# apache/tez

Hardware: NVIDIA H100
Metric: sorted KV GB/s (16B key / 64B val) (higher is better)
Workload: dtype u8

## Files before the change

### tez_b200/csrc/emit_fast.cuh

```cuda
#pragma once
#include "sorter_kernels.cuh"

#ifndef TEZGPU_EMIT_MIN_CTAS
#define TEZGPU_EMIT_MIN_CTAS 4
#endif

namespace tezgpu {

constexpr int FE_THREADS = 256;
constexpr int FE_MAX_RECS = 256;
constexpr int FE_IMG_BYTES = 22016;

struct TileDesc {
  uint32_t p;
  uint32_t r0;
  uint32_t nr;
  uint32_t flags;
  uint64_t abs0;
  uint64_t after;
};

struct TileCrc {
  uint32_t raw;
  uint32_t p;
  uint64_t after;
};

__global__ void k_build_tiles(EmitParams e, TileDesc *__restrict__ tiles) {
  uint32_t tile = blockIdx.x * blockDim.x + threadIdx.x;
  if (tile >= e.tile_start[e.P]) return;
  int lo = 0, hi = e.P;
  while (hi - lo > 1) {
    int mid = (lo + hi) >> 1;
    if (e.tile_start[mid] <= tile) lo = mid; else hi = mid;
  }
  const uint32_t p = (uint32_t)lo;
  const uint32_t ps = e.part_start[p], pe = e.part_start[p + 1];
  const uint32_t k = tile - e.tile_start[p];
  TileDesc d;
  d.p = p;
  d.r0 = ps + k * e.recs_per_tile;
  d.nr = min(e.recs_per_tile, pe - d.r0);
  const bool first = (k == 0), last = (d.r0 + d.nr == pe);
  d.flags = (first ? 1u : 0u) | (last ? 2u : 0u);
  const uint64_t seg0 = e.seg_start[p];
  d.abs0 = seg0 + (first ? 0 : 4 + (uint64_t)(d.r0 - ps) * e.rec_size);
  const uint64_t tile_end = seg0 + 4 + (uint64_t)(d.r0 - ps + d.nr) * e.rec_size + (last ? 2 : 0);
  d.after = (e.seg_start[p + 1] - 4) - tile_end;
  tiles[tile] = d;
}

__global__ void k_crc_combine(const TileCrc *__restrict__ tc, uint32_t ntiles, const CrcTables *__restrict__ t,
                              uint32_t *__restrict__ seg_crc) {
  uint32_t i = blockIdx.x * blockDim.x + threadIdx.x;
  const int lane = threadIdx.x & 31;
  uint32_t p = 0xFFFFFFFFu, val = 0;
  if (i < ntiles) {
    TileCrc c = tc[i];
    p = c.p;
    val = c.raw ? crc_shift_bytes(t, c.raw, c.after) : 0u;
  }
#pragma unroll
  for (int o = 1; o < 32; o <<= 1) {
    uint32_t v2 = __shfl_up_sync(0xffffffffu, val, o), p2 = __shfl_up_sync(0xffffffffu, p, o);
    if (lane >= o && p2 == p) val ^= v2;
  }
  uint32_t pn = __shfl_down_sync(0xffffffffu, p, 1);
  if (p != 0xFFFFFFFFu && (lane == 31 || pn != p) && val) atomicXor(&seg_crc[p], val);
}

__device__ __forceinline__ void sts_b8(uint32_t a, uint32_t v) { asm volatile("st.shared.b8 [%0], %1;" ::"r"(a), "r"(v) : "memory"); }
__device__ __forceinline__ void sts_b16(uint32_t a, uint32_t v) { asm volatile("st.shared.b16 [%0], %1;" ::"r"(a), "h"((unsigned short)v) : "memory"); }
// ... 32 lines not shown

__device__ __forceinline__ uint4 ldg_stream_v4(const void *p) {
  uint4 r;
  asm volatile("ld.global.nc.L1::no_allocate.v4.u32 {%0,%1,%2,%3}, [%4];"
               : "=r"(r.x), "=r"(r.y), "=r"(r.z), "=r"(r.w) : "l"(p));
  return r;
}
__device__ __forceinline__ void stg_stream_v4(void *p, uint4 v) {
  asm volatile("st.global.L1::no_allocate.v4.u32 [%0], {%1,%2,%3,%4};" ::"l"(p), "r"(v.x), "r"(v.y), "r"(v.z), "r"(v.w) : "memory");
}

struct FastEmitParams {
  EmitParams e;
  const TileDesc *tiles;
  TileCrc *tile_crc;
  uint32_t ntiles;
  uint32_t cpr;
  uint32_t cpr_magic;
  uint32_t stride;
};

__device__ __forceinline__ uint64_t fast_source_offset(const Records &rec, uint32_t ri, uint32_t stride, uint32_t p) {
  if (rec.use_runs) return run_record_off_p(rec.runs, p, ri) + rec.runs.hdr_len;
  return rec.key_off ? rec.key_off[ri] : (uint64_t)ri * stride;
}

template <int UNROLL, bool ALIGNED>
__global__ void __launch_bounds__(FE_THREADS, TEZGPU_EMIT_MIN_CTAS) k_emit_fast(FastEmitParams fp) {
  __shared__ __align__(16) uint8_t s_img[FE_IMG_BYTES];
  __shared__ uint32_t s_idx[2][FE_MAX_RECS];
  __shared__ uint64_t s_off[ALIGNED ? 1 : 2][ALIGNED ? 1 : FE_MAX_RECS];
// ... 5 lines not shown
  const int tid = threadIdx.x, lane = tid & 31, warp = tid >> 5;
  for (int i = tid; i < 4 * 256; i += FE_THREADS) {
    s_tab[i] = (&e.crc->slice[0][0])[i];
    s_adv32[i] = (&e.crc->adv128[0][0])[i];
  }
  const uint32_t lane_pow = e.crc->pow_word[4 * (31 - lane)];
  WarpLinearMap m_word, m_skip;
  {
    const uint32_t *gt = &e.crc->slice[0][0], *ga = &e.crc->advc[0][0];
    m_word.init([&](uint32_t x) { return gt[768 + (x & 0xFF)] ^ gt[512 + ((x >> 8) & 0xFF)] ^ gt[256 + ((x >> 16) & 0xFF)] ^ gt[x >> 24]; }, lane);
    m_skip.init([&](uint32_t x) { return ga[x & 0xFF] ^ ga[256 + ((x >> 8) & 0xFF)] ^ ga[512 + ((x >> 16) & 0xFF)] ^ ga[768 + (x >> 24)]; }, lane);
  }
  const uint32_t img_base = (uint32_t)__cvta_generic_to_shared(s_img);
  const uint8_t *__restrict__ kv = e.rec.kv;
  const uint8_t *kv_end = kv + e.rec.kv_bytes;
  const uint32_t rec_size = e.rec_size, hdr_len = e.fixed_hdr_len, stride = fp.stride;

  TileDesc td_next;
  if (blockIdx.x < fp.ntiles) {
    td_next = fp.tiles[blockIdx.x];
    if ((uint32_t)tid < td_next.nr) {
      const uint32_t ri = e.order[td_next.r0 + tid];
      s_idx[0][tid] = ri;
      if (!ALIGNED) s_off[0][tid] = fast_source_offset(e.rec, ri, stride, td_next.p);
    }
  }
  uint32_t buf = 0;
  for (uint32_t tile = blockIdx.x; tile < fp.ntiles; tile += gridDim.x, buf ^= 1u) {
    const TileDesc td = td_next;
    const uint32_t nr = td.nr;
    const bool first_tile = td.flags & 1u, last_tile = td.flags & 2u;
    const uint32_t tile_n = tile + gridDim.x;
    if (tile_n < fp.ntiles) td_next = fp.tiles[tile_n];
    __syncthreads();
    const uint32_t *__restrict__ c_idx = s_idx[buf];
    const uint64_t *__restrict__ c_off = s_off[ALIGNED ? 0 : buf];
    const uint64_t abs0 = td.abs0;
    const uint32_t lead = (uint32_t)(abs0 & 15u);
    const uint32_t rec0 = lead + (first_tile ? 4u : 0u);
    const uint32_t body_end = rec0 + nr * rec_size + (last_tile ? 2u : 0u);

    const uint32_t npieces = nr * fp.cpr;
    const uint32_t half_up = (nr + 1) >> 1;
    for (uint32_t q0 = tid; q0 < npieces; q0 += FE_THREADS * UNROLL) {
      uint4 v[UNROLL];
      uint32_t dst[UNROLL];
#pragma unroll
      for (int u = 0; u < UNROLL; u++) {
// ... 18 lines not shown
              case 2: w0 = lo4.z; w1 = lo4.w; w2 = hi4.x; w3 = hi4.y; w4 = hi4.z; break;
              default: w0 = lo4.w; w1 = hi4.x; w2 = hi4.y; w3 = hi4.z; w4 = hi4.w; break;
            }
            v[u] = make_uint4(__funnelshift_r(w0, w1, bsh), __funnelshift_r(w1, w2, bsh), __funnelshift_r(w2, w3, bsh),
                              __funnelshift_r(w3, w4, bsh));
          }
          dst[u] = img_base + rec0 + j * rec_size + hdr_len + 16u * c;
        }
      }
#pragma unroll
      for (int u = 0; u < UNROLL; u++) {
        uint32_t q = q0 + u * FE_THREADS;
        if (q < npieces) sts16_unaligned(dst[u], v[u]);
      }
    }
    if (tile_n < fp.ntiles && (uint32_t)tid < td_next.nr) {
      const uint32_t ri = e.order[td_next.r0 + tid];
      s_idx[buf ^ 1u][tid] = ri;
      if (!ALIGNED) s_off[buf ^ 1u][tid] = fast_source_offset(e.rec, ri, stride, td_next.p);
    }
    if ((uint32_t)tid < nr) {
      uint32_t a = img_base + rec0 + tid * rec_size;
      for (uint32_t b = 0; b < hdr_len; b++) sts_b8(a + b, e.fixed_hdr[b]);
    }
    if (tid == 0) {
      if (first_tile) { s_img[lead] = 'T'; s_img[lead + 1] = 'I'; s_img[lead + 2] = 'F'; s_img[lead + 3] = 0; }
      if (last_tile) { s_img[body_end - 2] = 0xFF; s_img[body_end - 1] = 0xFF; }
    }
    __syncthreads();

    const uint32_t cb0 = rec0, cb1 = body_end;
// ... 71 lines not shown
```

### tez_b200/csrc/emit_pipe.cuh

```cuda
#pragma once
#include "emit_fast.cuh"

#ifndef TEZGPU_EMIT4_MIN_CTAS
#define TEZGPU_EMIT4_MIN_CTAS 3
#endif

namespace tezgpu {

constexpr int FE4_BATCH = FE_THREADS / 32;
constexpr int FE4_UNROLL = 5;
constexpr int FE4_RUN = 5;
constexpr uint32_t FE4_RUN_BYTES = 16u * FE4_RUN;
constexpr int FE4_IMG_BYTES = FE_THREADS * FE4_RUN * 16;
constexpr int FE4_GROUPS = 2;
constexpr int FE4_PARKED = 4;
constexpr int FE4_WBITS = 7;
constexpr int FE4_WDIGITS = (32 + FE4_WBITS - 1) / FE4_WBITS;
constexpr int FE4_WENTRIES = ((FE4_WDIGITS - 1) << FE4_WBITS) + (1 << (32 - FE4_WBITS * (FE4_WDIGITS - 1)));

static inline uint32_t emit4_max_recs(uint32_t rec_size) {
  return std::min<uint32_t>(FE_MAX_RECS, (FE4_IMG_BYTES - 15 - 4 - 2) / rec_size);
}

constexpr uint32_t FE4_MAX_CPR = 8;
// ... 47 lines not shown
  using L = Emit4Smem;
  constexpr int BATCH = FE4_PARKED;
  extern __shared__ __align__(16) uint8_t smem4[];
  uint32_t *s_wtab = reinterpret_cast<uint32_t *>(smem4);
  uint32_t *s_tab = reinterpret_cast<uint32_t *>(smem4 + L::WTAB);
  uint32_t *s_hor = s_tab + 256;
  const int sub = threadIdx.x / FE_THREADS, tid = threadIdx.x % FE_THREADS, lane = tid & 31, warp = tid >> 5;
  uint8_t *gbase = smem4 + L::SHARED + (size_t)sub * L::GROUP;
  uint8_t *s_img = gbase;
  uint32_t(*s_idx)[FE_MAX_RECS] = reinterpret_cast<uint32_t(*)[FE_MAX_RECS]>(gbase + FE4_IMG_BYTES);
  uint32_t(*s_part)[FE_THREADS] = reinterpret_cast<uint32_t(*)[FE_THREADS]>(gbase + FE4_IMG_BYTES + 3 * FE_MAX_RECS * 4);
  FoldMeta *s_meta = reinterpret_cast<FoldMeta *>(gbase + FE4_IMG_BYTES + 3 * FE_MAX_RECS * 4 + (size_t)BATCH * FE_THREADS * 4);
  auto group_sync = [&]() { asm volatile("bar.sync %0, %1;" ::"r"(sub + 1), "r"(FE_THREADS) : "memory"); };

  const EmitParams &e = fp.e;
  const uint32_t G = gridDim.x * FE4_GROUPS, ntiles = fp.ntiles;
  uint32_t tile = blockIdx.x * FE4_GROUPS + sub;
  for (int i = threadIdx.x; i < FE4_WENTRIES * 32; i += FE_THREADS * FE4_GROUPS)
    s_wtab[i] = emit4_wtab_value(e.crc, (uint32_t)(i >> 5) >> FE4_WBITS, (uint32_t)(i >> 5) & ((1u << FE4_WBITS) - 1));
  for (int i = threadIdx.x; i < 256; i += FE_THREADS * FE4_GROUPS) s_tab[i] = e.crc->slice[0][i];
  {
    const uint32_t x_hor = e.crc->pow0[FE4_RUN_BYTES * 32];
    for (int i = threadIdx.x; i < 4 * 256; i += FE_THREADS * FE4_GROUPS) s_hor[i] = crc_multmodp((uint32_t)(i & 255) << (8 * (i >> 8)), x_hor);
  }
  __syncthreads();
  if (tile >= ntiles) return;
  const uint32_t lane_pow = e.crc->pow0[FE4_RUN_BYTES * (31 - lane)];
  const uint8_t *wt = reinterpret_cast<const uint8_t *>(s_wtab + lane);
  auto next_word = [&](uint32_t x) -> uint32_t { return emit4_next_word(wt, x); };
  const uint32_t img_base = (uint32_t)__cvta_generic_to_shared(s_img);
  const uint8_t *__restrict__ kv = e.rec.kv;
// ... 191 lines not shown
```

### tez_b200/csrc/emit_pipe_u.cuh

```cuda
#pragma once
#include "emit_pipe.cuh"

namespace tezgpu {

struct Emit4uSmem {
  static constexpr size_t SHARED = 256 * 4 + 4 * 256 * 4;
  static constexpr size_t TOTAL = SHARED + FE_IMG_BYTES + 3 * FE_MAX_RECS * 8 + (size_t)FE4_BATCH * FE_THREADS * 4 + (size_t)FE4_BATCH * sizeof(FoldMeta);
};

constexpr int FE4U_UNROLL = 5;
static inline uint32_t emit4u_max_recs(uint32_t cpr) {
  const uint32_t w = cpr + 1;
  return w > 32 ? 0u : (uint32_t)FE4U_UNROLL * (FE_THREADS / 32) * (32u / w);
}

__device__ __forceinline__ uint4 window16(uint4 lo, uint4 hi, uint32_t sh) {
  uint32_t w0 = lo.x, w1 = lo.y, w2 = lo.z, w3 = lo.w, w4 = hi.x, w5 = hi.y, w6 = hi.z, w7 = hi.w;
  if (sh & 4u) { w0 = w1; w1 = w2; w2 = w3; w3 = w4; w4 = w5; w5 = w6; w6 = w7; }
  if (sh & 8u) { w0 = w2; w1 = w3; w2 = w4; w3 = w5; w4 = w6; }
  const uint32_t bsh = (sh & 3u) * 8u;
  return make_uint4(__funnelshift_r(w0, w1, bsh), __funnelshift_r(w1, w2, bsh), __funnelshift_r(w2, w3, bsh), __funnelshift_r(w3, w4, bsh));
}

template <int UNROLL>
__global__ void __launch_bounds__(FE_THREADS, TEZGPU_EMIT4_MIN_CTAS) k_emit_fast4u(FastEmitParams fp) {
  constexpr int BATCH = FE4_BATCH;
  extern __shared__ __align__(16) uint8_t smem4u[];
  uint32_t *s_tab = reinterpret_cast<uint32_t *>(smem4u);
  uint32_t *s_adv128 = s_tab + 256;
  uint8_t *s_img = smem4u + Emit4uSmem::SHARED;
  uint64_t(*s_off)[FE_MAX_RECS] = reinterpret_cast<uint64_t(*)[FE_MAX_RECS]>(s_img + FE_IMG_BYTES);
  uint32_t(*s_part)[FE_THREADS] = reinterpret_cast<uint32_t(*)[FE_THREADS]>(s_img + FE_IMG_BYTES + 3 * FE_MAX_RECS * 8);
  FoldMeta *s_meta = reinterpret_cast<FoldMeta *>(s_img + FE_IMG_BYTES + 3 * FE_MAX_RECS * 8 + (size_t)BATCH * FE_THREADS * 4);

  const EmitParams &e = fp.e;
  const int tid = threadIdx.x, lane = tid & 31, warp = tid >> 5;
  const uint32_t G = gridDim.x, ntiles = fp.ntiles;
  uint32_t tile = blockIdx.x;
  if (tile >= ntiles) return;
  s_tab[tid] = e.crc->slice[0][tid];
  for (int i = tid; i < 4 * 256; i += FE_THREADS) s_adv128[i] = (&e.crc->adv128[0][0])[i];
  CrcChunkFoldT<false> cf;
  cf.init(e.crc, lane);
  const uint32_t lane_pow = cf.lane_pow;
  const uint32_t img_base = (uint32_t)__cvta_generic_to_shared(s_img);
  const uint8_t *__restrict__ kv = e.rec.kv;
  const uint8_t *kv_end = kv + e.rec.kv_bytes;
  const uint64_t *__restrict__ key_off = e.rec.key_off;
  const uint32_t rec_size = e.rec_size, hdr_len = e.fixed_hdr_len, stride = fp.stride, cpr = fp.cpr;
  const TileDesc *__restrict__ tiles = fp.tiles;
  const bool use_runs = e.rec.use_runs;
  auto source_offset = [&](uint32_t ri, uint32_t p) -> uint64_t {
// ... 215 lines not shown
```

### tez_b200/csrc/sorter.cuh

```cuda
#pragma once
#include <stddef.h>
#include <stdlib.h>
#include <string.h>

#include <memory>
#include <mutex>
#include <vector>

#include "../../include/tezgpu.h"
#include "device_util.h"
#include "combine.cuh"
#include "emit_pipe_u.cuh"
#include "sorter_kernels.cuh"

namespace tezgpu {

__global__ void k_store_to_host(uint32_t *__restrict__ dst0, const uint32_t *__restrict__ src0, uint32_t n0, uint32_t *__restrict__ dst1,
                                const uint32_t *__restrict__ src1, uint32_t n1, uint32_t *__restrict__ dst2,
                                const uint32_t *__restrict__ src2, uint32_t n2) {
  for (uint32_t i = threadIdx.x; i < n0; i += blockDim.x) dst0[i] = src0[i];
  for (uint32_t i = threadIdx.x; i < n1; i += blockDim.x) dst1[i] = src1[i];
  for (uint32_t i = threadIdx.x; i < n2; i += blockDim.x) dst2[i] = src2[i];
  __threadfence_system();
}
// ... 51 lines not shown
}

struct FramingMismatch {};

struct SortVerdict {
  int error;
  union { uint32_t large_groups; uint32_t batch_count; };
  unsigned long long dups;
  uint64_t totals[2];
};
struct SortScratch {
  uint32_t hist[8 * RADIX];
  uint32_t trivial[8];
  uint32_t tile_counter[8];
  SortVerdict verdict;
  uint32_t unused[2];
  unsigned long long ties;
};
constexpr size_t SORT_SCRATCH_BYTES = 16 * 1024;
struct SortHostScratch {
  SortVerdict verdict;
  uint32_t ties;
  uint64_t total;
  uint32_t trivial[8];
  static constexpr size_t INDEX_OFFSET = 4096;
  int64_t *index() { return reinterpret_cast<int64_t *>(reinterpret_cast<uint8_t *>(this) + INDEX_OFFSET); }
};
static_assert(offsetof(SortScratch, trivial) == 2048 * 4 && offsetof(SortScratch, tile_counter) == 2056 * 4 &&
                  offsetof(SortScratch, verdict) == 2064 * 4 && sizeof(SortVerdict) == 32 && offsetof(SortScratch, ties) == 2074 * 4 &&
                  sizeof(SortScratch) <= SORT_SCRATCH_BYTES && offsetof(SortHostScratch, ties) == 32 &&
                  sizeof(SortHostScratch) <= SortHostScratch::INDEX_OFFSET, "sort scratch layout");

enum class FixedEmitKernel {
  Pipe,
  Fast,
  PipeUnaligned,
  FastUnaligned,
  General,
};
struct FixedEmitPlan {
  FixedEmitKernel kernel;
  uint32_t recs_per_tile;
};

static inline FixedEmitPlan plan_fixed_emit(const Records &rec, uint32_t rec_size) {
  const uint32_t stride = rec.klen + rec.vlen, cpr = stride / 16;
  const uint32_t cap = std::max<uint32_t>(1, std::min<uint32_t>(EMIT_MAX_RECS, (FE_IMG_BYTES - 32) / rec_size));
// ... 56 lines not shown
    if (stream) cudaStreamDestroy(stream);
  }

  static uint64_t output_bound(uint64_t n, uint64_t kv_bytes, int P) { return kv_bytes + 12 * n + 10ull * P + 64; }

  SortScratch *d_scratch() const { return small.as<SortScratch>(); }
  SortHostScratch *h_scratch() const { return h_small.as<SortHostScratch>(); }

  struct SortState {
    Records rec;
    uint32_t *K = nullptr;
    uint32_t *order = nullptr;
    uint64_t dup_count = 0, tie_records = 0;
    int launches = 0;
    bool have_bounds = false, spec_layout = false;
    const uint8_t *same = nullptr;
  } state;
  int merge_check_same = 1;
  bool merge_inputs_plain = false;
  int combiner = TEZGPU_COMBINE_NONE;
  DeviceBuffer sp_prefix, sp_len, sp_off, sp_blob;
  SplitTable splits{};
  bool have_splits = false;
  void set_split_points(const HostSplitTable &t) {
    const size_t n = t.prefix.size();
    sp_prefix.ensure(std::max<size_t>(n, 1) * 8);
    sp_len.ensure(std::max<size_t>(n, 1) * 4);
    sp_off.ensure(std::max<size_t>(n, 1) * 8);
    sp_blob.ensure(std::max<size_t>(t.blob.size(), 16));
    if (n) {
// ... 32 lines not shown
    return e;
  }
  FixedEmitKernel set_fixed_layout(EmitParams &e, const Records &rec) {
    const FixedFraming f = fixed_framing(rec.klen, rec.vlen);
    memcpy(e.fixed_hdr, f.bytes, f.len);
    e.fixed_hdr_len = f.len;
    e.rec_size = f.rec_size;
    const FixedEmitPlan plan = plan_fixed_emit(rec, e.rec_size);
    e.recs_per_tile = plan.recs_per_tile;
    e.rec_off = nullptr;
    return plan.kernel;
  }

  void run(Records rec, uint8_t *d_out, uint64_t out_cap, uint64_t *out_len, int64_t *index, tezgpu_stats *stats) {
    const uint64_t raw_bound = output_bound(rec.n, rec.fixed ? (uint64_t)rec.n * (rec.klen + rec.vlen) : rec.kv_bytes, conf.num_partitions);
    sort_phase(rec);
    int rle;
    if (conf.rle_policy == TEZGPU_RLE_ON) rle = 1;
    else if (conf.rle_policy == TEZGPU_RLE_OFF) rle = 0;
    else rle = (conf.sorter_impl == 1) ? 0 : ((double)state.dup_count > 0.1 * (double)rec.n);
    if (conf.sorter_impl == TEZGPU_SORTER_UNORDERED) rle = 0;
    emit_out(rle, false, raw_bound, d_out, out_cap, out_len, index, stats);
  }

  int codec = TEZGPU_CODEC_NONE;
  DeviceBuffer z_img, z_slots, z_csize, z_cadler, z_coff, z_segs, z_descs, z_pstart, z_tc, z_crc;
  PinnedBuffer z_host;
  EventTimer z_timer;
  static uint64_t codec_bound(int codec, uint64_t raw_bound, int P);
  void compress_image(const int64_t *raw_index, uint8_t *d_out, uint64_t out_cap, uint64_t *out_len, int64_t *index, tezgpu_stats *stats);

  void emit_out(int rle, bool merge_mode, uint64_t raw_bound, uint8_t *d_out, uint64_t out_cap, uint64_t *out_len, int64_t *index,
                tezgpu_stats *stats) {
    if (!codec) {
      if (combiner) emit_combined(rle, d_out, out_cap, out_len, index, stats);
      else emit_phase(rle, merge_mode, d_out, out_cap, out_len, index, stats);
      return;
    }
    const int P = conf.num_partitions;
    z_img.ensure(raw_bound + 64);
    std::vector<int64_t> raw_index((size_t)P * 3, 0);
    uint64_t raw_len = 0;
    tezgpu_stats st;
    memset(&st, 0, sizeof(st));
    if (combiner) emit_combined(rle, z_img.as<uint8_t>(), z_img.cap, &raw_len, raw_index.data(), &st);
    else emit_phase(rle, merge_mode, z_img.as<uint8_t>(), z_img.cap, &raw_len, raw_index.data(), &st);
    compress_image(raw_index.data(), d_out, out_cap, out_len, index, &st);
    if (stats) *stats = st;
  }

  void sort_phase(Records rec) {
    const uint32_t n = rec.n;
    const int P = conf.num_partitions;
    TG_CHECK(n <= RADIX_MAX_N, TEZGPU_E_INVALID, "more than 2^30-1 records in one sort");
    rec.cmp = conf.comparator;
    rec.hash_partition = conf.partitioner == TEZGPU_PART_HASH;
    rec.num_partitions = P;
    rec.pbits = pbits;
    rec.unordered = conf.sorter_impl == TEZGPU_SORTER_UNORDERED ? 1 : 0;
    TG_CHECK(rec.hash_partition || rec.partition || rec.use_runs || stage_splits().n || n == 0 || P == 1, TEZGPU_E_INVALID,
             "partition ids required (partitioner=GIVEN)");
    state.have_bounds = state.spec_layout = false;
    state.same = nullptr;
    timer.reset();
    timer.mark(stream);

    const size_t n4 = (size_t)(n ? n : 1) * 4;
    sortA.ensure(2 * n4); sortB.ensure(2 * n4);
    same.ensure(n ? n : 1);
    blk.ensure((div_up(n ? n : 1, SCAN_TILE) + 2) * 8);
    part_start.ensure(((size_t)P + 1) * 4);
    seg_start.ensure(((size_t)P + 1) * 8);
    tile_start.ensure(((size_t)P + 1) * 4);
    d_index.ensure((size_t)P * 24);
    seg_crc.ensure((size_t)P * 4);
    h_small.ensure(SortHostScratch::INDEX_OFFSET + (size_t)P * 24);

    TG_CUDA(cudaMemsetAsync(small.p, 0, SORT_SCRATCH_BYTES, stream));
    TG_CUDA(cudaMemsetAsync(seg_crc.p, 0, (size_t)P * 4, stream));

    state.K = sortA.as<uint32_t>();
    state.order = sortA.as<uint32_t>() + n;
    state.dup_count = state.tie_records = 0;
    int launches = 0;
    if (n) {
      uint32_t depth0;
      launches += alphabet_table(rec, &depth0);
      launches += stage_and_sort(rec);
      launches += fix_ties(rec, depth0);
      if (h_scratch()->verdict.large_groups) launches += refine_large_groups(rec, depth0);
    }
    timer.mark(stream);
    state.rec = rec;
    state.launches = launches;
  }

  int alphabet_table(Records &rec, uint32_t *depth) {
    *depth = (uint32_t)((32 - pbits) / 8);
    if (rec.fixed || rec.unordered || (getenv("TEZGPU_NO_SYM") && atoi(getenv("TEZGPU_NO_SYM")))) return 0;
    sym_sets.ensure(SYM_MAX_POS * 8 * 4);
    sym_tab.ensure(sizeof(SymTable));
    TG_CUDA(cudaMemsetAsync(sym_sets.p, 0, SYM_MAX_POS * 8 * 4, stream));
    k_symbols<<<(int)std::min<uint64_t>(div_up(rec.n, 256), (uint64_t)num_sms * 8), 256, 0, stream>>>(rec, sym_sets.as<uint32_t>());
    uint32_t hs[SYM_MAX_POS * 8];
    TG_CUDA(cudaMemcpyAsync(hs, sym_sets.p, sizeof(hs), cudaMemcpyDeviceToHost, stream));
    TG_CUDA(cudaStreamSynchronize(stream));
    SymTable *t = new SymTable();
// ... 38 lines not shown
    if (rec.unordered) {
      pass_mask = 0;
      for (int q = 0; q < 4; q++) if (8 * q + 8 > 32 - pbits) pass_mask |= 1u << q;
      if (!pass_mask) pass_mask = 1;
    }
    const int done = radix_sort_pairs(stream, ws, sortA.as<uint32_t>(), sortB.as<uint32_t>(), n, 0, 4, pass_mask, &launches);
    if (done & 1) { state.K = sortB.as<uint32_t>(); state.order = sortB.as<uint32_t>() + n; }
    if (rec.unordered) {
      k_flip_order<<<(uint32_t)div_up(n, 256), 256, 0, stream>>>(state.order, n);
      launches++;
    }
    timer.mark(stream);
    return launches;
  }

  int fix_ties(const Records &rec, uint32_t depth0) {
    const uint32_t n = rec.n;
    const int P = conf.num_partitions;
    SortScratch *d = d_scratch();
    SortHostScratch *h = h_scratch();
    int per_sm_tf = 0;
    TG_CUDA(cudaOccupancyMaxActiveBlocksPerMultiprocessor(&per_sm_tf, k_tie_fix, TIEFIX_THREADS, 0));
    if (!rec.unordered)
      k_tie_fix<<<(uint32_t)std::min<uint64_t>(div_up(n, TIEFIX_TILE), (uint64_t)num_sms * std::max(per_sm_tf, 1)), TIEFIX_THREADS, 0, stream>>>(
          rec, state.K, state.order, n, depth0, same.as<uint8_t>(), &d->verdict.dups, &d->verdict.large_groups, &d->ties);
    k_part_bounds<<<(uint32_t)div_up((uint64_t)P + 1, 256), 256, 0, stream>>>(state.K, n, P, pbits, part_start.as<uint32_t>());
    int launches = 2;
    state.have_bounds = true;
    if (rec.fixed) {
      EmitParams e = make_emit_params(rec, state.order, 0, false, nullptr);
      set_fixed_layout(e, rec);
      k_layout<<<1, 1024, 0, stream>>>(e, seg_start.as<uint64_t>(), tile_start.as<uint32_t>(), d_index.as<int64_t>(), d->verdict.totals);
      launches++;
      state.spec_layout = true;
    }
    TG_CUDA(cudaGetLastError());
    store_to_host(stream, &h->verdict, &d->verdict, sizeof(SortVerdict), &h->ties, &d->ties, 4, h->index(), d_index.p,
                  state.spec_layout ? (size_t)P * 24 : 0);
    TG_CUDA(cudaGetLastError());
    TG_CUDA(cudaStreamSynchronize(stream));
    TG_CHECK(!(h->verdict.error & STAGE_ERR_PARTITION), TEZGPU_E_INVALID, "Illegal partition (outside [0, numPartitions))");
    if (h->verdict.error & STAGE_ERR_FRAMING) throw FramingMismatch();
    state.tie_records = h->ties;
    state.dup_count = h->verdict.dups;
    return launches;
  }

  int refine_large_groups(const Records &rec, uint32_t depth0) {
    const uint32_t n = rec.n, nblk = (uint32_t)div_up(n, SCAN_TILE);
    SortScratch *d = d_scratch();
    SortHostScratch *h = h_scratch();
    int launches = 0;
    auto scan_total = [&](uint32_t nb) {
      k_scan_block_sums<<<1, 1024, 0, stream>>>(blk.as<uint64_t>(), nb);
      launches++;
      TG_CUDA(cudaGetLastError());
      TG_CUDA(cudaMemcpyAsync(&h->total, blk.as<uint64_t>() + nb, 8, cudaMemcpyDeviceToHost, stream));
      TG_CUDA(cudaStreamSynchronize(stream));
      return h->total;
// ... 61 lines not shown
      }
    }
    TG_CUDA(cudaMemcpyAsync(&h->total, &d->verdict.dups, 8, cudaMemcpyDeviceToHost, stream));
    TG_CUDA(cudaStreamSynchronize(stream));
    state.dup_count = h->total;
    return launches;
  }

  void emit_phase(int rle, bool merge_mode, uint8_t *d_out, uint64_t out_cap, uint64_t *out_len, int64_t *index,
                  tezgpu_stats *stats) {
    TG_CHECK(((uintptr_t)d_out & 15u) == 0, TEZGPU_E_INVALID, "output buffer must be 16-byte aligned");
    const Records rec = state.rec;
    const uint32_t n = rec.n;
    const int P = conf.num_partitions;
    uint32_t *K = state.K, *order = state.order;
    const uint64_t dup_count = state.dup_count, tie_records = state.tie_records;
    int launches = state.launches;
    const CrcTables *d_crc = DeviceConstants::get(conf.device).d_crc;
    const size_t n4 = (size_t)(n ? n : 1) * 4;
    TG_CUDA(cudaMemsetAsync(seg_crc.p, 0, (size_t)P * 4, stream));
    if (timer.n > (n ? 4 : 2)) timer.n = n ? 4 : 2;

    EmitParams e = make_emit_params(rec, order, rle, merge_mode, d_out);
    if (!state.have_bounds) {
      k_part_bounds<<<(uint32_t)div_up((uint64_t)P + 1, 256), 256, 0, stream>>>(K, n, P, pbits, part_start.as<uint32_t>());
      launches++;
    }
    const bool no_repeats = !rle && (!merge_mode || (!merge_check_same && merge_inputs_plain));
    const bool fixed_emit = rec.fixed && (dup_count == 0 || no_repeats);
    uint64_t bound = output_bound(n, rec.fixed ? (uint64_t)n * (rec.klen + rec.vlen) : rec.kv_bytes, P);
    const FixedEmitKernel kernel = fixed_emit ? set_fixed_layout(e, rec) : FixedEmitKernel::General;
    if (!fixed_emit || !state.spec_layout) {
      if (!fixed_emit) {
// ... 14 lines not shown
        }
        e.rec_off = rec_off.as<uint64_t>();
      }
      k_layout<<<1, 1024, 0, stream>>>(e, seg_start.as<uint64_t>(), tile_start.as<uint32_t>(), d_index.as<int64_t>(), d_scratch()->verdict.totals);
      launches++;
      TG_CUDA(cudaGetLastError());
      store_to_host(stream, h_scratch()->verdict.totals, d_scratch()->verdict.totals, 16, h_scratch()->index(), d_index.p, (size_t)P * 24);
      TG_CUDA(cudaGetLastError());
      TG_CUDA(cudaStreamSynchronize(stream));
      state.spec_layout = false;
    }
    const uint64_t file_bytes = h_scratch()->verdict.totals[0];
    const uint64_t tiles = h_scratch()->verdict.totals[1];
    TG_CHECK(file_bytes <= bound, TEZGPU_E_INVALID, "internal: output exceeds bound");
    TG_CHECK(file_bytes <= out_cap, TEZGPU_E_NOMEM, "output buffer too small for file.out");
    const bool source_oriented = fixed_emit && kernel != FixedEmitKernel::General;
    const uint32_t stride = rec.klen + rec.vlen;
    FastEmitParams fp;
    if (tiles && source_oriented) {
      tile_desc.ensure((size_t)tiles * sizeof(TileDesc));
      k_build_tiles<<<(uint32_t)div_up(tiles, 256), 256, 0, stream>>>(e, tile_desc.as<TileDesc>());
      launches++;
      fp.e = e;
      tile_crc.ensure((size_t)tiles * sizeof(TileCrc));
      fp.tile_crc = tile_crc.as<TileCrc>();
      fp.tiles = tile_desc.as<TileDesc>();
      fp.ntiles = (uint32_t)tiles;
      fp.cpr = stride / 16;
      fp.cpr_magic = fp.cpr == 1 ? 0u : (uint32_t)((1ull << 32) / fp.cpr) + 1u;
      fp.stride = stride;
    }
    timer.mark(stream);
    if (tiles) {
      auto persistent_grid = [&](auto kern, int threads, size_t smem) {
        int per_sm = 0;
        TG_CUDA(cudaOccupancyMaxActiveBlocksPerMultiprocessor(&per_sm, kern, threads, smem));
        return (uint32_t)std::min<uint64_t>(tiles, (uint64_t)num_sms * (per_sm > 0 ? per_sm : 1));
      };
      if (!fixed_emit) {
        k_emit<false><<<persistent_grid(k_emit<false>, EMIT_THREADS, 0), EMIT_THREADS, 0, stream>>>(e);
      } else {
        switch (kernel) {
// ... 8 lines not shown
            break;
          case FixedEmitKernel::PipeUnaligned:
            set_smem_limit<k_emit_fast4u<FE4U_UNROLL>>(conf.device, Emit4uSmem::TOTAL);
            k_emit_fast4u<FE4U_UNROLL><<<persistent_grid(k_emit_fast4u<FE4U_UNROLL>, FE_THREADS, Emit4uSmem::TOTAL), FE_THREADS,
                                         Emit4uSmem::TOTAL, stream>>>(fp);
            break;
          case FixedEmitKernel::FastUnaligned:
            k_emit_fast<5, false><<<persistent_grid(k_emit_fast<5, false>, FE_THREADS, 0), FE_THREADS, 0, stream>>>(fp);
            break;
          case FixedEmitKernel::General:
            k_emit<true><<<persistent_grid(k_emit<true>, EMIT_THREADS, 0), EMIT_THREADS, 0, stream>>>(e);
            break;
        }
      }
      if (source_oriented) {
        k_crc_combine<<<(uint32_t)div_up(tiles, 256), 256, 0, stream>>>(fp.tile_crc, (uint32_t)tiles, d_crc, seg_crc.as<uint32_t>());
        launches++;
      }
      launches++;
      TG_CUDA(cudaGetLastError());
    }
    timer.mark(stream);
    k_finalize_segments<<<(uint32_t)div_up(P, 256), 256, 0, stream>>>(e);
    launches++;
    TG_CUDA(cudaGetLastError());
    timer.mark(stream);
    TG_CUDA(cudaStreamSynchronize(stream));

    if (out_len) *out_len = file_bytes;
    const int64_t *hidx = h_scratch()->index();
    if (index) memcpy(index, hidx, (size_t)P * 24);
    if (stats) {
      memset(stats, 0, sizeof(*stats));
      stats->output_records = n;
      int64_t raw = 0;
      for (int p = 0; p < P; p++) raw += hidx[3 * p + 1];
      stats->output_bytes_with_overhead = raw;
      stats->output_bytes_physical = (int64_t)file_bytes;
      stats->file_out_bytes = (int64_t)file_bytes;
      stats->spilled_records = n;
      stats->num_spills = 1;
      stats->rle_used = rle;
      stats->adjacent_equal_keys = (int64_t)dup_count;
      stats->tie_records = (int64_t)tie_records;
      const int b = n ? 3 : 1;
      stats->ms_stage = n ? timer.ms(0, 1) : 0;
      stats->ms_sort = n ? timer.ms(1, 2) : 0;
      stats->ms_ties = n ? timer.ms(2, 3) : 0;
      stats->ms_emit = timer.ms(b, b + 3);
      stats->ms_emit_kernel = timer.ms(b + 1, b + 2);
      stats->ms_total = timer.ms(0, b + 3);
      stats->kernel_launches = launches;
    }
  }

  bool combine_phase() {
    const Records rec = state.rec;
    const uint32_t n = rec.n, W = combine_width(combiner);
    TG_CHECK(W, TEZGPU_E_INVALID, "unknown combiner");
// ... 138 lines not shown
```

### tez_b200/csrc/sorter_kernels.cuh

```cuda
#pragma once
#include "common.cuh"
#include "crc32.cuh"
#include "radix_sort.cuh"
#include "scan.cuh"
#include "total_order.cuh"

namespace tezgpu {

struct RunTable {
  const uint64_t *seg_off;
  const uint32_t *rec_base;
  const uint32_t *seg_part;
  const uint32_t *part_seg0;
  uint32_t nseg;
  uint32_t rec_size;
  uint32_t hdr_len;
  uint64_t hdr_bytes[2];
};

__device__ __forceinline__ uint32_t run_of(const RunTable &t, uint32_t i) {
  uint32_t lo = 0, hi = t.nseg;
  while (hi - lo > 1) {
    const uint32_t mid = (lo + hi) >> 1;
    if (__ldg(t.rec_base + mid) <= i) lo = mid; else hi = mid;
// ... 416 lines not shown
    if (x != y) return x < y ? -1 : 1;
  }
  for (; i < nmin; i++) {
    uint32_t x = a[i], y = b[i];
    if (x != y) return x < y ? -1 : 1;
  }
  return la < lb ? -1 : (la == lb ? 0 : 1);
}

constexpr uint32_t TIE_SMALL_MAX = 16;

constexpr int TIEFIX_THREADS = 256;
constexpr int TIEFIX_IPT = 8;
constexpr int TIEFIX_TILE = TIEFIX_THREADS * TIEFIX_IPT;

constexpr int TIEFIX_FLUSH = 4 * TIEFIX_THREADS;
constexpr int TIEFIX_CAP = TIEFIX_FLUSH + TIEFIX_TILE / 2 + 8;

__device__ __forceinline__ void tie_fix_group(const Records &r, const uint32_t *__restrict__ K, uint32_t *__restrict__ order,
                                              uint32_t n, uint32_t i, uint32_t depth, uint8_t *__restrict__ same,
                                              uint32_t &my_dups, uint32_t &my_ties, uint32_t *__restrict__ large_groups) {
  const uint32_t k = K[i];
  uint32_t e = i + 2;
  while (e < n && e - i <= TIE_SMALL_MAX && K[e] == k) e++;
  const uint32_t sz = e - i;
  if (sz > TIE_SMALL_MAX) { atomicAdd(large_groups, 1u); return; }
  my_ties += sz;
  uint32_t idx[TIE_SMALL_MAX];
  for (uint32_t j = 0; j < sz; j++) idx[j] = order[i + j];
  uint32_t eq = 0;
// ... 168 lines not shown

__global__ void k_part_bounds(const uint32_t *__restrict__ K, uint32_t n, int P, int pbits,
                              uint32_t *__restrict__ part_start) {
  int p = blockIdx.x * blockDim.x + threadIdx.x;
  if (p > P) return;
  if (p == P) { part_start[p] = n; return; }
  if (pbits == 0) { part_start[p] = 0; return; }
  uint64_t target = (uint64_t)p << (32 - pbits);
  uint32_t lo = 0, hi = n;
  while (lo < hi) {
    uint32_t mid = lo + ((hi - lo) >> 1);
    if ((uint64_t)K[mid] < target) lo = mid + 1;
    else hi = mid;
  }
  part_start[p] = lo;
}

struct EmitParams {
  Records rec;
  const uint32_t *order;
  const uint8_t *same;
  const uint64_t *rec_off;
  const uint32_t *part_start;
  const uint64_t *seg_start;
  const uint32_t *tile_start;
  uint8_t *out;
  uint32_t *seg_crc;
  const CrcTables *crc;
  uint32_t recs_per_tile;
  uint32_t rec_size;
// ... 389 lines not shown
    for (uint32_t c = tid; c < nchunks; c += EMIT_THREADS) {
      uint32_t b0 = 16u * c, b1 = b0 + 16u;
      if (b0 >= lead && b1 <= lead + plen) {
        *reinterpret_cast<uint4 *>(dst + b0) = *reinterpret_cast<const uint4 *>(s_img + b0);
      } else {
        uint32_t a = max(b0, lead), b = min(b1, lead + plen);
        for (uint32_t x = a; x < b; x++) dst[x] = s_img[x];
      }
    }
    __syncthreads();
    done += plen;
  }
  }
}

__global__ void k_finalize_segments(EmitParams e) {
  int p = blockIdx.x * blockDim.x + threadIdx.x;
  if (p >= e.P) return;
  uint64_t s0 = e.seg_start[p], s1 = e.seg_start[p + 1];
  if (s1 == s0) return;
  uint32_t cnt = e.part_start[p + 1] - e.part_start[p];
  uint8_t *o = e.out + s0;
  uint32_t crc;
  if (cnt == 0) {
    o[0] = 'T'; o[1] = 'I'; o[2] = 'F'; o[3] = 0; o[4] = 0xFF; o[5] = 0xFF;
    crc = 0xFFFF0000u;
    o += 6;
  } else {
    crc = crc_from_raw(e.crc, e.seg_crc[p], s1 - s0 - 8);
    o += s1 - s0 - 4;
  }
  store_be32(o, crc);
}
// ... 3 lines not shown
```

Baseline: 536.4.

## Speculatively launch fixed-record emit before host verdict sync, gated on device

Result: no change. 537.8, median of 6 (+0.3%).

```diff
diff --git a/tez_b200/csrc/emit_fast.cuh b/tez_b200/csrc/emit_fast.cuh
--- a/tez_b200/csrc/emit_fast.cuh
+++ b/tez_b200/csrc/emit_fast.cuh
@@ -26,9 +26,9 @@
   uint64_t after;
 };
 
-__global__ void k_build_tiles(EmitParams e, TileDesc *__restrict__ tiles) {
+__global__ void k_build_tiles(EmitParams e, TileDesc *__restrict__ tiles, const uint32_t *__restrict__ ntiles) {
   uint32_t tile = blockIdx.x * blockDim.x + threadIdx.x;
-  if (tile >= e.tile_start[e.P]) return;
+  if (tile >= *ntiles) return;
   int lo = 0, hi = e.P;
   while (hi - lo > 1) {
     int mid = (lo + hi) >> 1;
@@ -51,11 +51,11 @@
 }
 
 __global__ void k_crc_combine(const TileCrc *__restrict__ tc, uint32_t ntiles, const CrcTables *__restrict__ t,
-                              uint32_t *__restrict__ seg_crc) {
+                              uint32_t *__restrict__ seg_crc, const uint32_t *__restrict__ dev_ntiles = nullptr) {
   uint32_t i = blockIdx.x * blockDim.x + threadIdx.x;
   const int lane = threadIdx.x & 31;
   uint32_t p = 0xFFFFFFFFu, val = 0;
-  if (i < ntiles) {
+  if (i < (dev_ntiles ? *dev_ntiles : ntiles)) {
     TileCrc c = tc[i];
     p = c.p;
     val = c.raw ? crc_shift_bytes(t, c.raw, c.after) : 0u;
@@ -118,7 +118,7 @@
   EmitParams e;
   const TileDesc *tiles;
   TileCrc *tile_crc;
-  uint32_t ntiles;
+  const uint32_t *ntiles;
   uint32_t cpr;
   uint32_t cpr_magic;
   uint32_t stride;
@@ -154,10 +154,10 @@
   const uint32_t img_base = (uint32_t)__cvta_generic_to_shared(s_img);
   const uint8_t *__restrict__ kv = e.rec.kv;
   const uint8_t *kv_end = kv + e.rec.kv_bytes;
-  const uint32_t rec_size = e.rec_size, hdr_len = e.fixed_hdr_len, stride = fp.stride;
+  const uint32_t rec_size = e.rec_size, hdr_len = e.fixed_hdr_len, stride = fp.stride, ntiles = *fp.ntiles;
 
   TileDesc td_next;
-  if (blockIdx.x < fp.ntiles) {
+  if (blockIdx.x < ntiles) {
     td_next = fp.tiles[blockIdx.x];
     if ((uint32_t)tid < td_next.nr) {
       const uint32_t ri = e.order[td_next.r0 + tid];
@@ -166,12 +166,12 @@
     }
   }
   uint32_t buf = 0;
-  for (uint32_t tile = blockIdx.x; tile < fp.ntiles; tile += gridDim.x, buf ^= 1u) {
+  for (uint32_t tile = blockIdx.x; tile < ntiles; tile += gridDim.x, buf ^= 1u) {
     const TileDesc td = td_next;
     const uint32_t nr = td.nr;
     const bool first_tile = td.flags & 1u, last_tile = td.flags & 2u;
     const uint32_t tile_n = tile + gridDim.x;
-    if (tile_n < fp.ntiles) td_next = fp.tiles[tile_n];
+    if (tile_n < ntiles) td_next = fp.tiles[tile_n];
     __syncthreads();
     const uint32_t *__restrict__ c_idx = s_idx[buf];
     const uint64_t *__restrict__ c_off = s_off[ALIGNED ? 0 : buf];
@@ -220,7 +220,7 @@
         if (q < npieces) sts16_unaligned(dst[u], v[u]);
       }
     }
-    if (tile_n < fp.ntiles && (uint32_t)tid < td_next.nr) {
+    if (tile_n < ntiles && (uint32_t)tid < td_next.nr) {
       const uint32_t ri = e.order[td_next.r0 + tid];
       s_idx[buf ^ 1u][tid] = ri;
       if (!ALIGNED) s_off[buf ^ 1u][tid] = fast_source_offset(e.rec, ri, stride, td_next.p);
diff --git a/tez_b200/csrc/emit_pipe.cuh b/tez_b200/csrc/emit_pipe.cuh
--- a/tez_b200/csrc/emit_pipe.cuh
+++ b/tez_b200/csrc/emit_pipe.cuh
@@ -85,7 +85,7 @@
   auto group_sync = [&]() { asm volatile("bar.sync %0, %1;" ::"r"(sub + 1), "r"(FE_THREADS) : "memory"); };
 
   const EmitParams &e = fp.e;
-  const uint32_t G = gridDim.x * FE4_GROUPS, ntiles = fp.ntiles;
+  const uint32_t G = gridDim.x * FE4_GROUPS, ntiles = *fp.ntiles;
   uint32_t tile = blockIdx.x * FE4_GROUPS + sub;
   for (int i = threadIdx.x; i < FE4_WENTRIES * 32; i += FE_THREADS * FE4_GROUPS)
     s_wtab[i] = emit4_wtab_value(e.crc, (uint32_t)(i >> 5) >> FE4_WBITS, (uint32_t)(i >> 5) & ((1u << FE4_WBITS) - 1));
diff --git a/tez_b200/csrc/emit_pipe_u.cuh b/tez_b200/csrc/emit_pipe_u.cuh
--- a/tez_b200/csrc/emit_pipe_u.cuh
+++ b/tez_b200/csrc/emit_pipe_u.cuh
@@ -35,7 +35,7 @@
 
   const EmitParams &e = fp.e;
   const int tid = threadIdx.x, lane = tid & 31, warp = tid >> 5;
-  const uint32_t G = gridDim.x, ntiles = fp.ntiles;
+  const uint32_t G = gridDim.x, ntiles = *fp.ntiles;
   uint32_t tile = blockIdx.x;
   if (tile >= ntiles) return;
   s_tab[tid] = e.crc->slice[0][tid];
diff --git a/tez_b200/csrc/sorter.cuh b/tez_b200/csrc/sorter.cuh
--- a/tez_b200/csrc/sorter.cuh
+++ b/tez_b200/csrc/sorter.cuh
@@ -89,7 +89,8 @@
   uint32_t trivial[8];
   uint32_t tile_counter[8];
   SortVerdict verdict;
-  uint32_t unused[2];
+  uint32_t spec_tiles;
+  uint32_t unused;
   unsigned long long ties;
 };
 constexpr size_t SORT_SCRATCH_BYTES = 16 * 1024;
@@ -106,6 +107,25 @@
                   sizeof(SortScratch) <= SORT_SCRATCH_BYTES && offsetof(SortHostScratch, ties) == 32 &&
                   sizeof(SortHostScratch) <= SortHostScratch::INDEX_OFFSET, "sort scratch layout");
 
+__host__ __device__ inline int rle_decision(int policy, int sorter_impl, uint64_t dups, uint32_t n) {
+  if (sorter_impl == TEZGPU_SORTER_UNORDERED || policy == TEZGPU_RLE_OFF) return 0;
+  if (policy == TEZGPU_RLE_ON) return 1;
+  return sorter_impl == 1 ? 0 : ((double)dups > 0.1 * (double)n);
+}
+
+struct SpecEmitCond {
+  uint32_t n;
+  int rle_policy, sorter_impl;
+  uint64_t out_cap, bound;
+};
+__host__ __device__ inline bool spec_emit_holds(const SortVerdict &v, const SpecEmitCond &c) {
+  return !v.error && !v.large_groups && (v.dups == 0 || !rle_decision(c.rle_policy, c.sorter_impl, v.dups, c.n)) &&
+         v.totals[0] <= c.out_cap && v.totals[0] <= c.bound;
+}
+__global__ void k_spec_gate(const SortVerdict *__restrict__ v, SpecEmitCond c, uint32_t *__restrict__ gate) {
+  *gate = spec_emit_holds(*v, c) ? (uint32_t)v->totals[1] : 0u;
+}
+
 enum class FixedEmitKernel {
   Pipe,
   Fast,
@@ -192,6 +212,7 @@
     uint64_t dup_count = 0, tie_records = 0;
     int launches = 0;
     bool have_bounds = false, spec_layout = false;
+    bool spec_emitted = false;
     const uint8_t *same = nullptr;
   } state;
   int merge_check_same = 1;
@@ -254,13 +275,12 @@
 
   void run(Records rec, uint8_t *d_out, uint64_t out_cap, uint64_t *out_len, int64_t *index, tezgpu_stats *stats) {
     const uint64_t raw_bound = output_bound(rec.n, rec.fixed ? (uint64_t)rec.n * (rec.klen + rec.vlen) : rec.kv_bytes, conf.num_partitions);
-    sort_phase(rec);
-    int rle;
-    if (conf.rle_policy == TEZGPU_RLE_ON) rle = 1;
-    else if (conf.rle_policy == TEZGPU_RLE_OFF) rle = 0;
-    else rle = (conf.sorter_impl == 1) ? 0 : ((double)state.dup_count > 0.1 * (double)rec.n);
-    if (conf.sorter_impl == TEZGPU_SORTER_UNORDERED) rle = 0;
-    emit_out(rle, false, raw_bound, d_out, out_cap, out_len, index, stats);
+    const SpecTarget spec{d_out, out_cap};
+    const bool speculate = rec.fixed && !codec && !combiner && ((uintptr_t)d_out & 15u) == 0;
+    sort_phase(rec, speculate ? &spec : nullptr);
+    const int rle = rle_decision(conf.rle_policy, conf.sorter_impl, state.dup_count, rec.n);
+    if (state.spec_emitted) finish_emit(rle, state.launches, out_len, index, stats);
+    else emit_out(rle, false, raw_bound, d_out, out_cap, out_len, index, stats);
   }
 
   int codec = TEZGPU_CODEC_NONE;
@@ -289,7 +309,12 @@
     if (stats) *stats = st;
   }
 
-  void sort_phase(Records rec) {
+  struct SpecTarget {
+    uint8_t *out;
+    uint64_t out_cap;
+  };
+
+  void sort_phase(Records rec, const SpecTarget *spec = nullptr) {
     const uint32_t n = rec.n;
     const int P = conf.num_partitions;
     TG_CHECK(n <= RADIX_MAX_N, TEZGPU_E_INVALID, "more than 2^30-1 records in one sort");
@@ -300,7 +325,7 @@
     rec.unordered = conf.sorter_impl == TEZGPU_SORTER_UNORDERED ? 1 : 0;
     TG_CHECK(rec.hash_partition || rec.partition || rec.use_runs || stage_splits().n || n == 0 || P == 1, TEZGPU_E_INVALID,
              "partition ids required (partitioner=GIVEN)");
-    state.have_bounds = state.spec_layout = false;
+    state.have_bounds = state.spec_layout = state.spec_emitted = false;
     state.same = nullptr;
     timer.reset();
     timer.mark(stream);
@@ -327,10 +352,10 @@
       uint32_t depth0;
       launches += alphabet_table(rec, &depth0);
       launches += stage_and_sort(rec);
-      launches += fix_ties(rec, depth0);
+      launches += fix_ties(rec, depth0, spec);
       if (h_scratch()->verdict.large_groups) launches += refine_large_groups(rec, depth0);
     }
-    timer.mark(stream);
+    if (!state.spec_emitted) timer.mark(stream);
     state.rec = rec;
     state.launches = launches;
   }
@@ -399,7 +424,7 @@
     return launches;
   }
 
-  int fix_ties(const Records &rec, uint32_t depth0) {
+  int fix_ties(const Records &rec, uint32_t depth0, const SpecTarget *spec) {
     const uint32_t n = rec.n;
     const int P = conf.num_partitions;
     SortScratch *d = d_scratch();
@@ -407,17 +432,31 @@
     int per_sm_tf = 0;
     TG_CUDA(cudaOccupancyMaxActiveBlocksPerMultiprocessor(&per_sm_tf, k_tie_fix, TIEFIX_THREADS, 0));
     if (!rec.unordered)
-      k_tie_fix<<<(uint32_t)std::min<uint64_t>(div_up(n, TIEFIX_TILE), (uint64_t)num_sms * std::max(per_sm_tf, 1)), TIEFIX_THREADS, 0, stream>>>(
+      k_tie_fix<<<(uint32_t)std::min<uint64_t>(div_up(n, TIEFIX_TILE), (uint64_t)num_sms * std::min(std::max(per_sm_tf, 1), TIEFIX_CTAS_PER_SM)),
+                  TIEFIX_THREADS, 0, stream>>>(
           rec, state.K, state.order, n, depth0, same.as<uint8_t>(), &d->verdict.dups, &d->verdict.large_groups, &d->ties);
-    k_part_bounds<<<(uint32_t)div_up((uint64_t)P + 1, 256), 256, 0, stream>>>(state.K, n, P, pbits, part_start.as<uint32_t>());
+    if (pbits <= 8)
+      k_part_bounds_hist<<<(uint32_t)div_up((uint64_t)P + 1, 256), 256, 0, stream>>>(d->hist + 3 * RADIX, n, P, pbits, part_start.as<uint32_t>());
+    else
+      k_part_bounds<<<(uint32_t)div_up((uint64_t)P + 1, 256), 256, 0, stream>>>(state.K, n, P, pbits, part_start.as<uint32_t>());
     int launches = 2;
     state.have_bounds = true;
+    bool speculated = false;
+    SpecEmitCond cond{};
     if (rec.fixed) {
-      EmitParams e = make_emit_params(rec, state.order, 0, false, nullptr);
-      set_fixed_layout(e, rec);
+      EmitParams e = make_emit_params(rec, state.order, 0, false, spec ? spec->out : nullptr);
+      const FixedEmitKernel kernel = set_fixed_layout(e, rec);
       k_layout<<<1, 1024, 0, stream>>>(e, seg_start.as<uint64_t>(), tile_start.as<uint32_t>(), d_index.as<int64_t>(), d->verdict.totals);
       launches++;
       state.spec_layout = true;
+      if (spec && kernel != FixedEmitKernel::General) {
+        cond = SpecEmitCond{n, conf.rle_policy, conf.sorter_impl, spec->out_cap, output_bound(n, (uint64_t)n * (rec.klen + rec.vlen), P)};
+        timer.mark(stream);
+        k_spec_gate<<<1, 1, 0, stream>>>(&d->verdict, cond, &d->spec_tiles);
+        const uint64_t max_tiles = div_up(n, e.recs_per_tile) + (uint64_t)P;
+        launches += 1 + launch_emit(e, true, kernel, max_tiles, &d->spec_tiles, &d->spec_tiles);
+        speculated = true;
+      }
     }
     TG_CUDA(cudaGetLastError());
     store_to_host(stream, &h->verdict, &d->verdict, sizeof(SortVerdict), &h->ties, &d->ties, 4, h->index(), d_index.p,
@@ -428,6 +467,8 @@
     if (h->verdict.error & STAGE_ERR_FRAMING) throw FramingMismatch();
     state.tie_records = h->ties;
     state.dup_count = h->verdict.dups;
+    state.spec_emitted = speculated && spec_emit_holds(h->verdict, cond);
+    if (speculated && !state.spec_emitted) timer.n = 3;
     return launches;
   }
 
@@ -519,9 +560,8 @@
     const uint32_t n = rec.n;
     const int P = conf.num_partitions;
     uint32_t *K = state.K, *order = state.order;
-    const uint64_t dup_count = state.dup_count, tie_records = state.tie_records;
+    const uint64_t dup_count = state.dup_count;
     int launches = state.launches;
-    const CrcTables *d_crc = DeviceConstants::get(conf.device).d_crc;
     const size_t n4 = (size_t)(n ? n : 1) * 4;
     TG_CUDA(cudaMemsetAsync(seg_crc.p, 0, (size_t)P * 4, stream));
     if (timer.n > (n ? 4 : 2)) timer.n = n ? 4 : 2;
@@ -566,18 +606,29 @@
     const uint64_t tiles = h_scratch()->verdict.totals[1];
     TG_CHECK(file_bytes <= bound, TEZGPU_E_INVALID, "internal: output exceeds bound");
     TG_CHECK(file_bytes <= out_cap, TEZGPU_E_NOMEM, "output buffer too small for file.out");
+    launches += launch_emit(e, fixed_emit, kernel, tiles, tile_start.as<uint32_t>() + P, nullptr);
+    TG_CUDA(cudaStreamSynchronize(stream));
+    finish_emit(rle, launches, out_len, index, stats);
+  }
+
+  int launch_emit(const EmitParams &e, bool fixed_emit, FixedEmitKernel kernel, uint64_t tiles, const uint32_t *d_ntiles,
+                  const uint32_t *gate) {
+    const Records &rec = e.rec;
+    const int P = conf.num_partitions;
+    const CrcTables *d_crc = DeviceConstants::get(conf.device).d_crc;
+    int launches = 0;
     const bool source_oriented = fixed_emit && kernel != FixedEmitKernel::General;
     const uint32_t stride = rec.klen + rec.vlen;
     FastEmitParams fp;
     if (tiles && source_oriented) {
       tile_desc.ensure((size_t)tiles * sizeof(TileDesc));
-      k_build_tiles<<<(uint32_t)div_up(tiles, 256), 256, 0, stream>>>(e, tile_desc.as<TileDesc>());
+      k_build_tiles<<<(uint32_t)div_up(tiles, 256), 256, 0, stream>>>(e, tile_desc.as<TileDesc>(), d_ntiles);
       launches++;
       fp.e = e;
       tile_crc.ensure((size_t)tiles * sizeof(TileCrc));
       fp.tile_crc = tile_crc.as<TileCrc>();
       fp.tiles = tile_desc.as<TileDesc>();
-      fp.ntiles = (uint32_t)tiles;
+      fp.ntiles = d_ntiles;
       fp.cpr = stride / 16;
       fp.cpr_magic = fp.cpr == 1 ? 0u : (uint32_t)((1ull << 32) / fp.cpr) + 1u;
       fp.stride = stride;
@@ -616,19 +667,24 @@
         }
       }
       if (source_oriented) {
-        k_crc_combine<<<(uint32_t)div_up(tiles, 256), 256, 0, stream>>>(fp.tile_crc, (uint32_t)tiles, d_crc, seg_crc.as<uint32_t>());
+        k_crc_combine<<<(uint32_t)div_up(tiles, 256), 256, 0, stream>>>(fp.tile_crc, (uint32_t)tiles, d_crc, seg_crc.as<uint32_t>(), d_ntiles);
         launches++;
       }
       launches++;
       TG_CUDA(cudaGetLastError());
     }
     timer.mark(stream);
-    k_finalize_segments<<<(uint32_t)div_up(P, 256), 256, 0, stream>>>(e);
+    k_finalize_segments<<<(uint32_t)div_up(P, 256), 256, 0, stream>>>(e, gate);
     launches++;
     TG_CUDA(cudaGetLastError());
     timer.mark(stream);
-    TG_CUDA(cudaStreamSynchronize(stream));
-
+    return launches;
+  }
+
+  void finish_emit(int rle, int launches, uint64_t *out_len, int64_t *index, tezgpu_stats *stats) {
+    const uint32_t n = state.rec.n;
+    const int P = conf.num_partitions;
+    const uint64_t file_bytes = h_scratch()->verdict.totals[0];
     if (out_len) *out_len = file_bytes;
     const int64_t *hidx = h_scratch()->index();
     if (index) memcpy(index, hidx, (size_t)P * 24);
@@ -643,8 +699,8 @@
       stats->spilled_records = n;
       stats->num_spills = 1;
       stats->rle_used = rle;
-      stats->adjacent_equal_keys = (int64_t)dup_count;
-      stats->tie_records = (int64_t)tie_records;
+      stats->adjacent_equal_keys = (int64_t)state.dup_count;
+      stats->tie_records = (int64_t)state.tie_records;
       const int b = n ? 3 : 1;
       stats->ms_stage = n ? timer.ms(0, 1) : 0;
       stats->ms_sort = n ? timer.ms(1, 2) : 0;
diff --git a/tez_b200/csrc/sorter_kernels.cuh b/tez_b200/csrc/sorter_kernels.cuh
--- a/tez_b200/csrc/sorter_kernels.cuh
+++ b/tez_b200/csrc/sorter_kernels.cuh
@@ -454,6 +454,7 @@
 constexpr int TIEFIX_IPT = 8;
 constexpr int TIEFIX_TILE = TIEFIX_THREADS * TIEFIX_IPT;
 
+constexpr int TIEFIX_CTAS_PER_SM = 3;
 constexpr int TIEFIX_FLUSH = 4 * TIEFIX_THREADS;
 constexpr int TIEFIX_CAP = TIEFIX_FLUSH + TIEFIX_TILE / 2 + 8;
 
@@ -652,6 +653,13 @@
     else hi = mid;
   }
   part_start[p] = lo;
+}
+
+__global__ void k_part_bounds_hist(const uint32_t *__restrict__ hist_top, uint32_t n, int P, int pbits,
+                                   uint32_t *__restrict__ part_start) {
+  int p = blockIdx.x * blockDim.x + threadIdx.x;
+  if (p > P) return;
+  part_start[p] = p == P ? n : hist_top[(uint32_t)p << (8 - pbits)];
 }
 
 struct EmitParams {
@@ -1071,9 +1079,9 @@
   }
 }
 
-__global__ void k_finalize_segments(EmitParams e) {
+__global__ void k_finalize_segments(EmitParams e, const uint32_t *__restrict__ gate) {
   int p = blockIdx.x * blockDim.x + threadIdx.x;
-  if (p >= e.P) return;
+  if (p >= e.P || (gate && *gate == 0)) return;
   uint64_t s0 = e.seg_start[p], s1 = e.seg_start[p + 1];
   if (s1 == s0) return;
   uint32_t cnt = e.part_start[p + 1] - e.part_start[p];
```
